# Quillboltcode/VLM-CLIP

Measured on AMD Instinct MI355X. Metric: image-text pairs/sec, ViT-B/16 contrastive step, 1/2/4/8 GPUs; MFMA % peak, higher is better.
Workload: dtype bf16

## Files before the change

vlm-clip_amd/csrc/gemm.hip:

```cpp
#include "common.h"
#include "internal.h"
#include <algorithm>
#include <cstring>
#include <type_traits>
#include <cstdlib>

#include "gemm_common.h"

namespace {
using namespace cmg;

template <bool AK, bool BKM, typename OutT, int EPI>
__global__ __launch_bounds__(NTHR, 2) void gemm_bf16_kernel(GemmP p) {
  extern __shared__ __attribute__((aligned(16))) char smem[];
  const int t = threadIdx.x, lane = t & 63, wave = t >> 6;
  const int wm = wave >> 1, wn = wave & 1;
  const int tile = xcd_remap(blockIdx.x, p.ntiles);
  const int tm = tile / p.tiles_n, tn = tile - tm * p.tiles_n;
  const int m0 = tm * BM, n0 = tn * BN;
  const int kbeg = blockIdx.y * p.k_per_split;
  const int kend = min(p.K, kbeg + p.k_per_split);
  const int nk = (kend - kbeg + BK - 1) / BK;

  Stager<AK> sa;
// ... 938 lines not shown
  }
}

template <bool AK, bool BKM, typename OutT, int EPI>
void launch_bf16(const GemmP& p, int splits, hipStream_t s) {
  hipLaunchKernelGGL((gemm_bf16_kernel<AK, BKM, OutT, EPI>), dim3(p.ntiles, splits), dim3(NTHR), 65536, s, p);
}

template <bool AK, bool BKM, typename OutT, int EPI, bool BG, int VAR>
void launch256v(const GemmP& p, int splits, hipStream_t s, float* bias_grad) {
  (void)lds_optin((const void*)gemm256_kernel<AK, BKM, OutT, EPI, BG, VAR>, 131072);
  hipLaunchKernelGGL((gemm256_kernel<AK, BKM, OutT, EPI, BG, VAR>), dim3(p.ntiles * splits), dim3(NT2), 131072, s,
                     p, bias_grad);
}
template <bool AK, bool BKM, typename OutT, int EPI, bool BG, int PPV>
void launch_ppv(const GemmP& p, int splits, hipStream_t s, float* bias_grad) {
  (void)lds_optin((const void*)gemm_pp_kernel<AK, BKM, OutT, EPI, BG, PPV>, PP_S * PP_STAGE);
  hipLaunchKernelGGL((gemm_pp_kernel<AK, BKM, OutT, EPI, BG, PPV>), dim3(p.ntiles * splits), dim3(NT2),
                     PP_S * PP_STAGE, s, p, bias_grad);
}
int num_cus() {
  static int n[64] = {0};
  int dev = 0;
  (void)hipGetDevice(&dev);
  dev &= 63;
  if (!n[dev]) {
    int c = 0;
    if (hipDeviceGetAttribute(&c, hipDeviceAttributeMultiprocessorCount, dev) != hipSuccess || c <= 0) c = 256;
    n[dev] = c;
  }
  return n[dev];
}
#ifdef CLIPMI_GEMM_EXPERIMENTS
template <bool AK, bool BKM, typename OutT, int EPI>
void launch_pps(const GemmP& p, hipStream_t s) {
  (void)lds_optin((const void*)gemm_pps_kernel<AK, BKM, OutT, EPI>, PP_S * PP_STAGE);
  const int grid = std::min(p.ntiles, num_cus());
  hipLaunchKernelGGL((gemm_pps_kernel<AK, BKM, OutT, EPI>), dim3(grid), dim3(NT2), PP_S * PP_STAGE, s, p);
}
template <bool BKM, typename OutT, int EPI>
void launch_hp(const GemmP& p, hipStream_t s) {
  (void)lds_optin((const void*)gemm_hp_kernel<BKM, OutT, EPI>, 131072);
  hipLaunchKernelGGL((gemm_hp_kernel<BKM, OutT, EPI>), dim3(p.ntiles), dim3(NT2), 131072, s, p);
}
#endif
template <bool AK, bool BKM, typename OutT, int EPI, bool BG>
void launch256(const GemmP& p, int splits, hipStream_t s, float* bias_grad) {
#ifdef CLIPMI_GEMM_EXPERIMENTS
  if (p.var == 10 && !BG && !p.ws && splits == 1) {
    launch_pps<AK, BKM, OutT, EPI>(p, s);
    return;
  }
  if constexpr (AK && !BG) {
    if (p.var == 11 && !p.ws && splits == 1) {
      launch_hp<BKM, OutT, EPI>(p, s);
      return;
    }
  }
  switch (p.var) {
    case 2: launch256v<AK, BKM, OutT, EPI, BG, 0>(p, splits, s, bias_grad); return;
    case 3: launch256v<AK, BKM, OutT, EPI, BG, 2>(p, splits, s, bias_grad); return;
    case 12: launch_ppv<AK, BKM, OutT, EPI, BG, 8>(p, splits, s, bias_grad); return;
    case 13: launch_ppv<AK, BKM, OutT, EPI, BG, 16>(p, splits, s, bias_grad); return;
    case 14: launch_ppv<AK, BKM, OutT, EPI, BG, 20>(p, splits, s, bias_grad); return;
    case 15: launch_ppv<AK, BKM, OutT, EPI, BG, 32>(p, splits, s, bias_grad); return;
    case 16: launch_ppv<AK, BKM, OutT, EPI, BG, 64>(p, splits, s, bias_grad); return;
    case 5: launch_ppv<AK, BKM, OutT, EPI, BG, 1>(p, splits, s, bias_grad); return;
    case 6: launch_ppv<AK, BKM, OutT, EPI, BG, 2>(p, splits, s, bias_grad); return;
    case 7: launch_ppv<AK, BKM, OutT, EPI, BG, 3>(p, splits, s, bias_grad); return;
    case 8: launch_ppv<AK, BKM, OutT, EPI, BG, 4>(p, splits, s, bias_grad); return;
    default: break;
  }
#endif
  if (p.var == 4) launch256v<AK, BKM, OutT, EPI, BG, 3>(p, splits, s, bias_grad);
  else launch_ppv<AK, BKM, OutT, EPI, BG, 0>(p, splits, s, bias_grad);
}

constexpr int E_B = CLIPMI_EPI_BIAS, E_R = CLIPMI_EPI_RESID, E_Q = CLIPMI_EPI_QGELU, E_G = CLIPMI_EPI_GELU;
constexpr int E_P = CLIPMI_EPI_STORE_PRE, E_DQ = CLIPMI_EPI_DQGELU, E_DG = CLIPMI_EPI_DGELU, E_BETA = CLIPMI_EPI_BETA;
constexpr int E_DA = CLIPMI_EPI_STORE_DACT, E_MA = CLIPMI_EPI_MUL_AUX;

bool w4_x3() {
  const char* e = getenv("CLIPMI_GEMM_X3_W4");
  return !(e && e[0] == '0');
}

const char* dispatch256(const GemmP& p, int splits, hipStream_t s, bool f32o, int sel, int flags, float* bg) {
  if (sel == 0 && (p.ws || (f32o && flags == E_BETA))) {
    if (p.var == 28 || p.var == 32) {
      if (const char* l = dispatch_w4_wgrad(p, splits, s, flags, bg)) return l;
    }
    if (p.ws) {
      if (bg) launch256<false, false, float, 0, true>(p, splits, s, bg);
      else launch256<false, false, float, 0, false>(p, splits, s, bg);
      return "gemm256_wgrad_splitk";
    }
    if (bg) launch256<false, false, float, E_BETA, true>(p, splits, s, bg);
    else launch256<false, false, float, E_BETA, false>(p, splits, s, bg);
    return "gemm256_wgrad";
  }
  if (bg) return nullptr;
  const bool w4_pf = p.var == 0 && sel == 2 && (flags == E_MA || (flags == 0 && p.K <= 768));
  const bool w4_default = p.var == 0 && (p.K >= 1536 || flags == E_MA);
  if ((w4_default || w4_pf || p.var == 20 || (p.var >= 22 && p.var <= 25 && p.dbg) || p.var == 28 || p.var == 32) &&
      !f32o && !p.ws && splits == 1 && (sel == 3 || sel == 2)) {
    GemmP q = p;
    const int dm = (p.var == 32 || w4_pf) ? 102 : (p.var == 28 || w4_default) ? 100 : p.var >= 22 ? 21 - p.var : 1;
    if (const char* l = dispatch_w4(q, s, sel == 3, flags, dm)) return l;
  }
  if (f32o && !p.ws && splits == 1 && sel == 3) {
    if ((w4_default || p.var == 28) && (flags == E_B || flags == (E_B | E_R) || flags == 0 || (p.x3o && w4_x3()))) {
      if (const char* l = dispatch_w4_f32(p, s, flags, true)) return l;
    }
    switch (flags) {
      case E_B: launch256<true, true, float, E_B, false>(p, splits, s, bg); return "gemm256_fwd_bias_f32";
      case E_B | E_R: launch256<true, true, float, E_B | E_R, false>(p, splits, s, bg); return "gemm256_fwd_bias_resid_f32";
      case 0: launch256<true, true, float, 0, false>(p, splits, s, bg); return "gemm256_fwd_f32";
      case E_B | E_Q | E_DA: launch256<true, true, float, E_B | E_Q | E_DA, false>(p, splits, s, bg); return "gemm256_fwd_bias_qgelu_dact_f32";
      case E_B | E_Q: launch256<true, true, float, E_B | E_Q, false>(p, splits, s, bg); return "gemm256_fwd_bias_qgelu_f32";
      default: break;
    }
  }
  if (f32o && !p.ws && splits == 1 && sel == 2) {
    if ((w4_default || p.var == 28) && (flags == 0 || (p.x3o && w4_x3()))) {
      if (const char* l = dispatch_w4_f32(p, s, flags, false)) return l;
    }
    switch (flags) {
      case 0: launch256<true, false, float, 0, false>(p, splits, s, bg); return "gemm256_dgrad_f32";
      case E_MA: launch256<true, false, float, E_MA, false>(p, splits, s, bg); return "gemm256_dgrad_mulaux_f32";
      default: break;
    }
  }
  if (sel == 3 && !f32o) {
    switch (flags) {
      case E_B: launch256<true, true, bf16, E_B, false>(p, splits, s, bg); return "gemm256_fwd_bias";
      case E_B | E_R: launch256<true, true, bf16, E_B | E_R, false>(p, splits, s, bg); return "gemm256_fwd_bias_resid";
      case E_B | E_Q | E_P: launch256<true, true, bf16, E_B | E_Q | E_P, false>(p, splits, s, bg); return "gemm256_fwd_bias_qgelu_pre";
      case E_B | E_Q | E_DA: launch256<true, true, bf16, E_B | E_Q | E_DA, false>(p, splits, s, bg); return "gemm256_fwd_bias_qgelu_dact";
      case E_B | E_Q: launch256<true, true, bf16, E_B | E_Q, false>(p, splits, s, bg); return "gemm256_fwd_bias_qgelu";
      case 0: launch256<true, true, bf16, 0, false>(p, splits, s, bg); return "gemm256_fwd";
      default: break;
    }
  }
  if (sel == 2 && !f32o) {
    switch (flags) {
      case 0: launch256<true, false, bf16, 0, false>(p, splits, s, bg); return "gemm256_dgrad";
      case E_DQ: launch256<true, false, bf16, E_DQ, false>(p, splits, s, bg); return "gemm256_dgrad_dqgelu";
      case E_MA: launch256<true, false, bf16, E_MA, false>(p, splits, s, bg); return "gemm256_dgrad_mulaux";
      default: break;
    }
  }
  return nullptr;
}

const char* dispatch_bf16(const GemmP& p, int splits, hipStream_t s, bool f32o, int sel, int flags) {
  if (p.ws) {
    if (sel == 0) { launch_bf16<false, false, float, 0>(p, splits, s); return "gemm_wgrad_splitk"; }
    launch_bf16<true, true, float, -1>(p, splits, s);
    return "gemm_generic";
  }
  if (sel == 3 && !f32o) {
    switch (flags) {
      case E_B: launch_bf16<true, true, bf16, E_B>(p, splits, s); return "gemm_fwd_bias";
      case E_B | E_R: launch_bf16<true, true, bf16, E_B | E_R>(p, splits, s); return "gemm_fwd_bias_resid";
      case E_B | E_Q | E_P: launch_bf16<true, true, bf16, E_B | E_Q | E_P>(p, splits, s); return "gemm_fwd_bias_qgelu_pre";
      case E_B | E_Q: launch_bf16<true, true, bf16, E_B | E_Q>(p, splits, s); return "gemm_fwd_bias_qgelu";
// ... 239 lines not shown
            ((uintptr_t)d->residual % 16 == 0) && ((uintptr_t)d->aux % 16 == 0);
    p.vec8 = d->c_dtype == CLIPMI_BF16 && d->N % 8 == 0 && d->ldc % 8 == 0 && d->ldr % 8 == 0 && d->ldaux % 8 == 0 &&
             ((uintptr_t)d->C % 16 == 0) && ((uintptr_t)d->residual % 16 == 0) && ((uintptr_t)d->aux % 16 == 0) &&
             ((uintptr_t)d->bias % 16 == 0);
    const double flops = 2.0 * d->M * d->N * d->K;
    ProfScope ps(s, nullptr, 0.0);
    const char* label = dispatch_fp8(p, s, d->c_dtype == CLIPMI_F32, q8o, d->flags);
    if (!label) return clipmi_invalid("fp8 output: supported epilogue flags are bias + quick_gelu");
    ps.finish(label, flops);
    CLIPMI_CHECK_LAUNCH();
    return CLIPMI_OK;
  }
  const bool bf = d->ab_dtype == CLIPMI_BF16;
  CLIPMI_REQUIRE(bf || d->ab_dtype == CLIPMI_F32, "ab_dtype");
  if (d->M == 0 || d->N == 0) return CLIPMI_OK;
  CLIPMI_REQUIRE(bf == false || d->b_kmajor || d->N % 8 == 0, "row-major B needs N % 8 == 0");
  CLIPMI_REQUIRE(d->c_dtype == CLIPMI_F32 || d->c_dtype == CLIPMI_BF16, "c_dtype");

  if (bf) {
    CLIPMI_REQUIRE(!d->a_kmajor || d->K % 8 == 0, "k-major A needs K % 8 == 0");
    CLIPMI_REQUIRE(!d->b_kmajor || d->K % 8 == 0, "k-major B needs K % 8 == 0");
    CLIPMI_REQUIRE(d->a_kmajor || d->M % 8 == 0, "row-major A needs M % 8 == 0");
    CLIPMI_REQUIRE(d->a_kmajor || d->M >= 8, "M >= 8");
    CLIPMI_REQUIRE(((uintptr_t)d->A & 15) == 0 && ((uintptr_t)d->B & 15) == 0, "A/B must be 16-byte aligned");
    CLIPMI_REQUIRE((d->lda % 8) == 0 && (d->ldb % 8) == 0, "lda/ldb must be multiples of 8");
  }
  int splits = d->split_k > 1 ? d->split_k : 1;
  GemmP p;
  memset(&p, 0, sizeof(p));
  p.M = d->M; p.N = d->N; p.K = d->K;
  p.A = d->A; p.lda = d->lda; p.B = d->B; p.ldb = d->ldb;
  p.C = d->C; p.ldc = d->ldc; p.bias = d->bias; p.res = d->residual; p.ldr = d->ldr;
  p.aux = d->aux; p.ldaux = d->ldaux; p.alpha = d->alpha; p.flags = d->flags;
  p.bias_f32 = d->bias_dtype == CLIPMI_F32;
  p.ws = nullptr;
  p.bws = nullptr;
  p.x3o = x3o;
  p.colp = colp;
  static const int env_var = [] {
    const char* e = getenv("CLIPMI_GEMM_VAR");
    return e ? atoi(e) : -1;
  }();
  static const int env_wvar = [] {
    const char* e = getenv("CLIPMI_GEMM_WVAR");
    return e ? atoi(e) : -1;
  }();
  const bool wlayout = !d->a_kmajor && !d->b_kmajor;
  const int evar = wlayout ? env_wvar : env_var;
  p.raster = raster_rows();
  p.dbg = gemm_stamp_buffer();
  p.stagger = 0;
  p.first_round = num_cus();
  if (d->force_small_tile >= 100 && d->force_small_tile < 200) {
    p.var = 9;
    p.stagger = d->force_small_tile % 100;
  } else if (d->force_small_tile >= 2) p.var = d->force_small_tile;
  else if (evar >= 0 && d->force_small_tile == 0) p.var = evar;
  else p.var = wlayout ? 28 : 0;
  p.vec = (d->ldc % 4 == 0) && (d->ldr % 4 == 0) && (d->ldaux % 4 == 0) && ((uintptr_t)d->C % 16 == 0) &&
          ((uintptr_t)d->residual % 16 == 0) && ((uintptr_t)d->aux % 16 == 0);
  p.vec8 = d->c_dtype == CLIPMI_BF16 && d->N % 8 == 0 && d->ldc % 8 == 0 && d->ldr % 8 == 0 && d->ldaux % 8 == 0 &&
           ((uintptr_t)d->C % 16 == 0) && ((uintptr_t)d->residual % 16 == 0) && ((uintptr_t)d->aux % 16 == 0) &&
           ((uintptr_t)d->bias % 16 == 0);
  const bool kok = (!d->a_kmajor || d->K % 64 == 0) && (!d->b_kmajor || d->K % 64 == 0);
  const bool use256 = bf && kok && ((d->M >= 256 && d->N >= 128) || d->bias_grad) && d->force_small_tile != 1;
  CLIPMI_REQUIRE(!d->bias_grad || use256, "bias_grad fusion needs the 256 kernel (bf16, wgrad layout)");
  CLIPMI_REQUIRE(!x3o || (use256 && splits == 1), "x3out: needs the 256-tile kernels (M >= 256, N >= 128, K % 64 == 0)");
  const int tile = bf ? (use256 ? BT : BM) : FT;
  const int kstep = bf ? BK : FK;
  if (splits > 1) {
    CLIPMI_REQUIRE(d->c_dtype == CLIPMI_F32, "split_k needs fp32 C");
    CLIPMI_REQUIRE((d->flags & ~CLIPMI_EPI_BETA) == 0, "split_k supports only the beta flag");
    CLIPMI_REQUIRE(d->workspace && d->workspace_bytes >= (int64_t)splits * d->M * (d->N + (d->bias_grad ? 1 : 0)) * 4,
                   "split_k workspace too small (split_k * M * (N + bias_grad ? 1 : 0) floats)");
    int per = (d->K + splits - 1) / splits;
    per = (per + kstep - 1) / kstep * kstep;
    splits = (d->K + per - 1) / per;
    p.k_per_split = per;
    p.ws = (float*)d->workspace;
    if (d->bias_grad) p.bws = p.ws + (int64_t)splits * d->M * d->N;
  } else {
    p.k_per_split = d->K > 0 ? d->K : 1;
  }
  p.tiles_n = (d->N + tile - 1) / tile;
  p.ntiles = p.tiles_n * ((d->M + tile - 1) / tile);
  const double flops = 2.0 * d->M * d->N * d->K;
  if (bf) {
    const bool f32o = d->c_dtype == CLIPMI_F32 || p.ws;
    const int sel = (d->a_kmajor ? 2 : 0) | (d->b_kmajor ? 1 : 0);
    ProfScope ps(s, nullptr, 0.0);
    const char* label = nullptr;
    if (use256) {
      GemmP q = p;
      q.tiles_n = (d->N + BT - 1) / BT;
      q.ntiles = q.tiles_n * ((d->M + BT - 1) / BT);
      if (wlayout && !getenv("CLIPMI_RASTER") && q.tiles_n > q.ntiles / q.tiles_n) q.raster = q.ntiles / q.tiles_n;
      label = dispatch256(q, splits, s, f32o, sel, d->flags, d->bias_grad);
      CLIPMI_REQUIRE(label || !x3o, "x3out: no image-output kernel for these flags");
    }
    if (!label) {
      CLIPMI_REQUIRE(!d->bias_grad, "bias_grad needs the wgrad layout (both operands row-major in k)");
      GemmP q = p;
      q.tiles_n = (d->N + BM - 1) / BM;
      q.ntiles = q.tiles_n * ((d->M + BM - 1) / BM);
      label = dispatch_bf16(q, splits, s, f32o, sel, d->flags);
    }
    CLIPMI_REQUIRE(label, "no kernel for this GEMM");
    ps.finish(label, flops);
  } else {
    ProfScope ps(s, nullptr, 0.0);
    if (d->c_dtype == CLIPMI_F32 || p.ws)
      hipLaunchKernelGGL(gemm_f32_kernel<float>, dim3(p.ntiles, splits), dim3(256), 0, s, p, d->a_kmajor, d->b_kmajor);
    else
      hipLaunchKernelGGL(gemm_f32_kernel<bf16>, dim3(p.ntiles, splits), dim3(256), 0, s, p, d->a_kmajor, d->b_kmajor);
    ps.finish("gemm_f32", flops);
  }
  CLIPMI_CHECK_LAUNCH();
  if (p.ws) {
    const int64_t total = (int64_t)d->M * d->N;
    const int beta = (d->flags & CLIPMI_EPI_BETA) ? 1 : 0;
    if (d->N % 4 == 0 && d->ldc % 4 == 0 && ((uintptr_t)d->C & 15) == 0 && ((uintptr_t)p.ws & 15) == 0) {
      DeferredReduce r;
      memset(&r, 0, sizeof(r));
      r.kind = 1;
      r.ws = p.ws; r.C = (float*)d->C; r.ldc = d->ldc; r.M = d->M; r.N = d->N; r.splits = splits;
      r.alpha = d->alpha; r.beta = beta; r.bws = p.bws; r.bias_grad = d->bias_grad;
      DeferredReduce* slot = deferred_slot();
      if (slot && slot->kind == 0) *slot = r;
      else CLIPMI_TRY(launch_deferred(s, r));
    } else {
      const unsigned nblk = (unsigned)std::min<int64_t>((total + 255) / 256, 8192);
      hipLaunchKernelGGL(splitk_reduce_kernel, dim3(nblk), dim3(256), 0, s,
                         p.ws, (float*)d->C, d->ldc, d->M, d->N, splits, d->alpha, beta);
      if (p.bws)
        hipLaunchKernelGGL(bias_partials_reduce_kernel, dim3((d->M + 255) / 256), dim3(256), 0, s, p.bws,
                           d->bias_grad, d->M, splits);
    }
    CLIPMI_CHECK_LAUNCH();
  }
  return CLIPMI_OK;
}
}

extern "C" int clipmi_gemm(void* stream, const clipmi_gemm_desc* d) { return gemm_impl(stream, d, 0, nullptr); }

namespace {
__global__ __launch_bounds__(256) void fold_rows4_kernel(const float* part, int P, int N, int per, float* out) {
  const int c = (blockIdx.x * 256 + threadIdx.x) * 4;
  if (c >= N) return;
  const int r0 = blockIdx.y * per, r1 = min(P, r0 + per);
  f32x4 acc = f32x4{0.f, 0.f, 0.f, 0.f};
  int r = r0;
  for (; r + 8 <= r1; r += 8) {
    f32x4 v[8];
#pragma unroll
    for (int j = 0; j < 8; ++j) v[j] = *(const f32x4*)(part + (int64_t)(r + j) * N + c);
#pragma unroll
    for (int j = 0; j < 8; ++j) acc += v[j];
  }
  for (; r < r1; ++r) acc += *(const f32x4*)(part + (int64_t)r * N + c);
  *(f32x4*)(out + (int64_t)blockIdx.y * N + c) = acc;
}
constexpr int X3_FOLD = 64;
int x3out_parts(int M) { return (M + 127) / 128; }
}

// ... 91 lines not shown
```

vlm-clip_amd/csrc/gemm_common.h:

```cpp
#pragma once
#include "common.h"
#include "internal.h"
#include <algorithm>
#include <type_traits>

namespace cmg {

constexpr int BM = 128, BN = 128, BK = 64, NTHR = 256;
constexpr int E8_B = CLIPMI_EPI_BIAS, E8_R = CLIPMI_EPI_RESID, E8_Q = CLIPMI_EPI_QGELU;

struct GemmP {
  int M, N, K;
  const void* A; int64_t lda;
  const void* B; int64_t ldb;
  void* C; int64_t ldc;
  const void* bias; const void* res; int64_t ldr;
  void* aux; int64_t ldaux;
  float alpha; int flags; int bias_f32;
  int k_per_split; float* ws;
  int tiles_n, ntiles;
  int vec;
  int var;
  int vec8;
  int stagger, first_round;
  const uint8_t* a_scale; const uint8_t* b_scale;
  uint8_t* c_scale;
  int raster;
  float* bws;
  unsigned long long* dbg;
  int* dyn;
  int nb2;
  int64_t bsa1, bsa2, bsb1, bsb2, bsc1, bsc2;
  DeferredReduce red;
  int x3o;
  float* colp;
};

unsigned long long* gemm_stamp_buffer();

__device__ __forceinline__ void tile_coords(const GemmP& p, int tile, int& tm, int& tn) {
  if (p.raster > 0) {
    const int g = p.raster, tiles_m = p.ntiles / p.tiles_n;
    const int grp = tile / (g * p.tiles_n);
    const int rem = tile - grp * g * p.tiles_n;
    const int rows = min(g, tiles_m - grp * g);
    tn = rem / rows;
    tm = grp * g + (rem - tn * rows);
  } else {
    tm = tile / p.tiles_n;
    tn = tile - tm * p.tiles_n;
  }
}

__device__ __forceinline__ float ld_bias(const GemmP& p, int n) {
  return p.bias_f32 ? ((const float*)p.bias)[n] : (float)((const bf16*)p.bias)[n];
}

template <typename OutT>
__device__ __forceinline__ void ld4(const OutT* p, float v[4], int nv, bool vec) {
  if (vec) { load4(p, v); return; }
#pragma unroll
  for (int j = 0; j < 4; ++j) v[j] = j < nv ? to_f32(p[j]) : 0.f;
}
template <typename OutT>
__device__ __forceinline__ void st4(OutT* p, const float v[4], int nv, bool vec) {
  if (vec) { store4(p, v); return; }
#pragma unroll
  for (int j = 0; j < 4; ++j)
    if (j < nv) p[j] = from_f32<OutT>(v[j]);
}

template <typename OutT, int EPI>
__device__ __forceinline__ void epilogue4(const GemmP& p, int m, int n, float v[4]) {
  const int f = EPI >= 0 ? EPI : p.flags;
  const int nv = min(4, p.N - n);
  const bool vec = p.vec && nv == 4;
#pragma unroll
  for (int j = 0; j < 4; ++j) v[j] *= p.alpha;
  if (f & CLIPMI_EPI_BIAS) {
#pragma unroll
    for (int j = 0; j < 4; ++j) v[j] += j < nv ? ld_bias(p, n + j) : 0.f;
  }
  if (f & CLIPMI_EPI_STORE_PRE) st4((OutT*)p.aux + (int64_t)m * p.ldaux + n, v, nv, vec);
  if (f & CLIPMI_EPI_STORE_DACT) {
    float d[4];
#pragma unroll
    for (int j = 0; j < 4; ++j) d[j] = (f & CLIPMI_EPI_QGELU) ? quick_gelu_grad(v[j]) : gelu_erf_grad(v[j]);
    st4((OutT*)p.aux + (int64_t)m * p.ldaux + n, d, nv, vec);
  }
  if (f & CLIPMI_EPI_QGELU) {
#pragma unroll
    for (int j = 0; j < 4; ++j) v[j] = quick_gelu(v[j]);
  } else if (f & CLIPMI_EPI_GELU) {
#pragma unroll
    for (int j = 0; j < 4; ++j) v[j] = gelu_erf(v[j]);
  }
  if (f & (CLIPMI_EPI_DQGELU | CLIPMI_EPI_DGELU)) {
    float a[4];
    ld4((const OutT*)p.aux + (int64_t)m * p.ldaux + n, a, nv, vec);
    if (f & CLIPMI_EPI_DQGELU) {
#pragma unroll
      for (int j = 0; j < 4; ++j) v[j] *= quick_gelu_grad(a[j]);
    } else {
#pragma unroll
      for (int j = 0; j < 4; ++j) v[j] *= gelu_erf_grad(a[j]);
    }
// ... 484 lines not shown
#pragma unroll
  for (int part = 0; part < NPART; ++part) {
    const int c = part >> 1, h = part & 1;
    u32x4 aux2[4][2];
#pragma unroll
    for (int ii = 0; ii < 4; ++ii) {
      const int i = h * 4 + ii;
#pragma unroll
      for (int jp = 0; jp < 2; ++jp) {
        float v[8];
        if constexpr (AR) __builtin_amdgcn_sched_barrier(0);
#pragma unroll
        for (int r = 0; r < 4; ++r) {
          const auto sw = __builtin_amdgcn_permlane16_swap(__float_as_uint(acc[c][i][2 * jp][r]),
                                                           __float_as_uint(acc[c][i][2 * jp + 1][r]), false, false);
          v[r] = __uint_as_float(sw[0]) * p.alpha + bv[c][jp][r];
          v[r + 4] = __uint_as_float(sw[1]) * p.alpha + bv[c][jp][r + 4];
        }
        float xin[8], w2[8];
        if (HIN) unpack8(xr[part % PD][ii][jp], xin);
#pragma unroll
        for (int r = 0; r < 8; ++r) {
          if (HPRE) w2[r] = v[r];
          if (HQ) {
            const float sg = qg_sigmoid(v[r]);
            if (HDA) {
              const float tq = 1.702f * v[r];
              w2[r] = fmaf(sg, fmaf(-tq, sg, tq), sg);
            }
            v[r] *= sg;
          }
          if (HG) {
            if (HDA) w2[r] = gelu_erf_grad(v[r]);
            v[r] = gelu_erf(v[r]);
          }
          if (HDQ) v[r] *= quick_gelu_grad(xin[r]);
          if (HDG) v[r] *= gelu_erf_grad(xin[r]);
          if (HMA) v[r] *= xin[r];
          if (HR || HBETA) v[r] += xin[r];
        }
        if (H2)
          aux2[ii][jp] = __builtin_bit_cast(u32x4, bf16x8{(bf16)w2[0], (bf16)w2[1], (bf16)w2[2], (bf16)w2[3],
                                                           (bf16)w2[4], (bf16)w2[5], (bf16)w2[6], (bf16)w2[7]});
        *LDS_PTR(bf16x8, st + stage_off(ii * 16 + mlane, (32 * jp + coff) >> 3)) =
            bf16x8{(bf16)v[0], (bf16)v[1], (bf16)v[2], (bf16)v[3], (bf16)v[4], (bf16)v[5], (bf16)v[6], (bf16)v[7]};
      }
    }
    if (HIN && part + PD < NPART) load_in(part + PD, xr[part % PD]);
    asm volatile("s_waitcnt lgkmcnt(0)" ::: "memory");
    u32x4 o[8];
#pragma unroll
    for (int it = 0; it < 8; ++it) o[it] = *LDS_PTR(const u32x4, st + stage_off(it * 8 + (lane >> 3), lane & 7));
    asm volatile("s_waitcnt lgkmcnt(0)" ::: "memory");
    if (H2) {
#pragma unroll
      for (int ii = 0; ii < 4; ++ii)
#pragma unroll
        for (int jp = 0; jp < 2; ++jp) *LDS_PTR(u32x4, st + stage_off(ii * 16 + mlane, (32 * jp + coff) >> 3)) = aux2[ii][jp];
    }
    const int r0 = mb + h * 64 + (lane >> 3), col = nb + 64 * c + (lane & 7) * 8;
    auto store_rows = [&](bf16* base, int64_t ld, const u32x4 (&rows)[8]) {
      bf16* out = base + (int64_t)r0 * ld + col;
      const int64_t step = 8 * ld;
      if (full) {
#pragma unroll
        for (int it = 0; it < 8; ++it) st16_out((u32x4*)(out + it * step), rows[it]);
      } else {
#pragma unroll
        for (int it = 0; it < 8; ++it)
          if (r0 + it * 8 < p.M && col < p.N) st16_out((u32x4*)(out + it * step), rows[it]);
      }
    };
    store_rows((bf16*)p.C, p.ldc, o);
    if (H2) {
      asm volatile("s_waitcnt lgkmcnt(0)" ::: "memory");
#pragma unroll
      for (int it = 0; it < 8; ++it) o[it] = *LDS_PTR(const u32x4, st + stage_off(it * 8 + (lane >> 3), lane & 7));
      asm volatile("s_waitcnt lgkmcnt(0)" ::: "memory");
      store_rows((bf16*)p.aux, p.ldaux, o);
    }
  }
}

template <int EPI, bool AR = false>
__device__ __forceinline__ void epilogue_x3img(const GemmP& p, f32x4 (&acc)[8][4], int mb, int nb, int lane) {
#pragma clang fp contract(off)
  constexpr bool HB = EPI & CLIPMI_EPI_BIAS, HQ = EPI & CLIPMI_EPI_QGELU;
  constexpr bool HDA = EPI & CLIPMI_EPI_STORE_DACT, HMA = EPI & CLIPMI_EPI_MUL_AUX;
  const int q = lane >> 4, mlane = lane & 15;
  const int coff = 16 * (q & 1) + 8 * (q >> 1);
  const int64_t seg = p.N;
  const bool p1 = p.x3o == 2;
  float bv[2][8];
#pragma unroll
  for (int jp = 0; jp < 2; ++jp) {
    const int n = min(nb + 32 * jp + coff, p.N - 8);
#pragma unroll
    for (int r = 0; r < 8; ++r) bv[jp][r] = 0.f;
    if (HB) {
      if (p.bias_f32) {
        load4((const float*)p.bias + n, bv[jp]);
        load4((const float*)p.bias + n + 4, bv[jp] + 4);
      } else {
        load8((const bf16*)p.bias + n, bv[jp]);
      }
    }
  }
  float cs[2][8];
#pragma unroll
  for (int jp = 0; jp < 2; ++jp)
#pragma unroll
    for (int r = 0; r < 8; ++r) cs[jp][r] = 0.f;
#pragma unroll
  for (int h = 0; h < 2; ++h) {
    float xin[4][2][8];
    if (HMA) {
#pragma unroll
      for (int ii = 0; ii < 4; ++ii) {
        const int m = min(mb + (h * 4 + ii) * 16 + mlane, p.M - 1);
#pragma unroll
        for (int jp = 0; jp < 2; ++jp) {
          const float* a = (const float*)p.aux + (int64_t)m * p.ldaux + min(nb + 32 * jp + coff, p.N - 8);
          load4(a, xin[ii][jp]);
          load4(a + 4, xin[ii][jp] + 4);
        }
      }
    }
#pragma unroll
    for (int ii = 0; ii < 4; ++ii) {
      const int i = h * 4 + ii;
      const int m = mb + i * 16 + mlane;
#pragma unroll
      for (int jp = 0; jp < 2; ++jp) {
        const int n = nb + 32 * jp + coff;
        float v[8], w2[8];
        if constexpr (AR) __builtin_amdgcn_sched_barrier(0);
#pragma unroll
        for (int r = 0; r < 4; ++r) {
          const auto sw = __builtin_amdgcn_permlane16_swap(__float_as_uint(acc[i][2 * jp][r]),
                                                           __float_as_uint(acc[i][2 * jp + 1][r]), false, false);
          v[r] = __uint_as_float(sw[0]) * p.alpha + bv[jp][r];
          v[r + 4] = __uint_as_float(sw[1]) * p.alpha + bv[jp][r + 4];
        }
#pragma unroll
        for (int r = 0; r < 8; ++r) {
          if (HQ) {
            const float sg = qg_sigmoid(v[r]);
            if (HDA) {
              const float tq = 1.702f * v[r];
              w2[r] = fmaf(sg, fmaf(-tq, sg, tq), sg);
            }
            v[r] *= sg;
          }
          if (HMA) v[r] *= xin[ii][jp][r];
        }
        if (m < p.M && n < p.N) {
          if (HDA) {
            float* a = (float*)p.aux + (int64_t)m * p.ldaux + n;
            store4(a, w2);
            store4(a + 4, w2 + 4);
          }
          bf16x8 hi, lo;
#pragma unroll
          for (int r = 0; r < 8; ++r) {
            hi[r] = (bf16)v[r];
            lo[r] = (bf16)(v[r] - (float)hi[r]);
            cs[jp][r] += v[r];
          }
          bf16* o = (bf16*)p.C + (int64_t)m * p.ldc + n;
          *(bf16x8*)o = hi;
          *(bf16x8*)(o + seg) = p1 ? lo : hi;
          *(bf16x8*)(o + 2 * seg) = p1 ? hi : lo;
        }
      }
    }
  }
  if (p.colp && mb < p.M) {
#pragma unroll
    for (int jp = 0; jp < 2; ++jp) {
#pragma unroll
      for (int r = 0; r < 8; ++r) {
#pragma unroll
        for (int o = 1; o < 16; o <<= 1) cs[jp][r] += __shfl_xor(cs[jp][r], o, 64);
      }
      const int n = nb + 32 * jp + coff;
      if (mlane == 0 && n < p.N) {
        float* c = p.colp + (int64_t)(mb >> 7) * p.N + n;
        store4(c, cs[jp]);
        store4(c + 4, cs[jp] + 4);
      }
    }
  }
}

template <typename OutT, int EPI, bool AR = false>
__device__ __forceinline__ void finish256(const GemmP& p, f32x4 (&acc)[8][4], int mb, int nb, int lane, int kz,
                                          char* stage = nullptr) {
  constexpr bool FAST = EPI >= 0 && !((EPI & CLIPMI_EPI_RESID) && (EPI & (CLIPMI_EPI_DQGELU | CLIPMI_EPI_DGELU))) &&
                        !((EPI & CLIPMI_EPI_BETA) && (EPI & (CLIPMI_EPI_RESID | CLIPMI_EPI_DQGELU | CLIPMI_EPI_DGELU)));
  constexpr int X3E = EPI & ~CLIPMI_EPI_STORE_DACT;
  if constexpr (std::is_same<OutT, float>::value &&
                (X3E == (CLIPMI_EPI_BIAS | CLIPMI_EPI_QGELU) || EPI == CLIPMI_EPI_MUL_AUX)) {
    if (p.x3o) {
      epilogue_x3img<EPI, AR>(p, acc, mb, nb, lane);
      return;
    }
  }
  constexpr bool NEWF = EPI >= 0 && (EPI & (CLIPMI_EPI_STORE_DACT | CLIPMI_EPI_MUL_AUX));
  if constexpr (NEWF) {
#if !CLIPMI_OLD_EPI
    if constexpr (std::is_same<OutT, bf16>::value) {
      if (stage && !p.ws && p.vec8) {
        epilogue_lds_pipe<EPI, AR, 1>(p, reinterpret_cast<f32x4(&)[1][8][4]>(acc), mb, nb, lane, stage);
        return;
      }
    }
#endif
  } else if constexpr (FAST && std::is_same<OutT, bf16>::value) {
    if (stage && !p.ws && p.vec8) {
#if CLIPMI_OLD_EPI
      epilogue256_lds<EPI < 0 ? 0 : EPI, AR>(p, acc, mb, nb, lane, stage);
#else
      epilogue_lds_pipe<EPI < 0 ? 0 : EPI, AR, 1>(p, reinterpret_cast<f32x4(&)[1][8][4]>(acc), mb, nb, lane, stage);
#endif
      return;
    }
    if (!p.ws && p.vec8) {
      epilogue256_w<EPI < 0 ? 0 : EPI, AR>(p, acc, mb, nb, lane);
      return;
    }
  }
  if (FAST && !NEWF && !p.ws && p.vec && (p.N & 3) == 0) {
    epilogue256<OutT, EPI < 0 ? 0 : EPI, AR>(p, acc, mb, nb, lane);
    return;
  }
#pragma unroll
  for (int i = 0; i < 8; ++i) {
    const int m = mb + i * 16 + (lane & 15);
    if (m >= p.M) continue;
#pragma unroll
    for (int j = 0; j < 4; ++j) {
      const int n = nb + j * 16 + (lane >> 4) * 4;
      if (n >= p.N) continue;
      acc_pin<AR>(acc[i][j]);
      float v[4] = {acc[i][j][0], acc[i][j][1], acc[i][j][2], acc[i][j][3]};
      if (p.ws) st4(p.ws + (int64_t)kz * p.M * p.N + (int64_t)m * p.N + n, v, min(4, p.N - n), p.vec && n + 4 <= p.N);
      else epilogue4<OutT, EPI>(p, m, n, v);
    }
  }
}

template <typename OutT, int EPI, bool AR>
__device__ __forceinline__ void finish256x2(const GemmP& p, f32x4 (&acc)[2][8][4], int mb, int nb, int lane, int kz,
                                            char* stage) {
  constexpr bool FAST = EPI >= 0 && !((EPI & CLIPMI_EPI_RESID) && (EPI & (CLIPMI_EPI_DQGELU | CLIPMI_EPI_DGELU))) &&
                        !((EPI & CLIPMI_EPI_BETA) && (EPI & (CLIPMI_EPI_RESID | CLIPMI_EPI_DQGELU | CLIPMI_EPI_DGELU)));
#if !CLIPMI_OLD_EPI
  if constexpr (FAST && std::is_same<OutT, bf16>::value) {
    if (stage && !p.ws && p.vec8) {
      epilogue_lds_pipe<EPI < 0 ? 0 : EPI, AR, 2>(p, acc, mb, nb, lane, stage);
      return;
    }
  }
#endif
  finish256<OutT, EPI, AR>(p, acc[0], mb, nb, lane, kz, stage);
  finish256<OutT, EPI, AR>(p, acc[1], mb, nb + 64, lane, kz, stage);
}

typedef __attribute__((ext_vector_type(8))) int i32x8;
typedef __attribute__((ext_vector_type(16))) float f32x16;
typedef __attribute__((ext_vector_type(2))) float f32x2;

template <int EPI, int NI = 8>
__device__ __forceinline__ void epilogue_q8(const GemmP& p, f32x4 (&acc)[NI][4], int mb, int nb, int lane) {
  constexpr bool HB = EPI & CLIPMI_EPI_BIAS, HQ = EPI & CLIPMI_EPI_QGELU, HG = EPI & CLIPMI_EPI_GELU;
  const int q = lane >> 4, mlane = lane & 15;
  const int coff = 16 * (q & 1) + 8 * (q >> 1);
  uint8_t* out = (uint8_t*)p.C;
  const int nsb = p.N >> 5;
  float bv[2][8];
#pragma unroll
  for (int jp = 0; jp < 2; ++jp) {
    const int n = min(nb + 32 * jp + coff, p.N - 8);
#pragma unroll
    for (int r = 0; r < 8; ++r) bv[jp][r] = 0.f;
    if (HB) {
      if (p.bias_f32) {
        load4((const float*)p.bias + n, bv[jp]);
        load4((const float*)p.bias + n + 4, bv[jp] + 4);
      } else {
        load8((const bf16*)p.bias + n, bv[jp]);
      }
    }
  }
#pragma unroll
  for (int i = 0; i < NI; ++i) {
    const int m = mb + i * 16 + mlane;
    uint32_t w[2][2];
    int ex[2];
#pragma unroll
    for (int jp = 0; jp < 2; ++jp) {
      f32x2 v2[4];
#pragma unroll
      for (int r = 0; r < 4; ++r) {
        const auto sw = __builtin_amdgcn_permlane16_swap(__float_as_uint(acc[i][2 * jp][r]),
                                                         __float_as_uint(acc[i][2 * jp + 1][r]), false, false);
        v2[r] = __builtin_elementwise_fma(f32x2{__uint_as_float(sw[0]), __uint_as_float(sw[1])},
                                          f32x2{p.alpha, p.alpha}, f32x2{bv[jp][r], bv[jp][r + 4]});
      }
      float am = 0.f;
#pragma unroll
      for (int r = 0; r < 4; ++r) {
        if (HQ) {
          const f32x2 z = v2[r] * f32x2{-1.702f * 1.4426950408889634f, -1.702f * 1.4426950408889634f};
          const f32x2 d = f32x2{__builtin_amdgcn_exp2f(z[0]), __builtin_amdgcn_exp2f(z[1])} + f32x2{1.0f, 1.0f};
          v2[r] = v2[r] * f32x2{__builtin_amdgcn_rcpf(d[0]), __builtin_amdgcn_rcpf(d[1])};
        }
        if (HG) v2[r] = f32x2{gelu_erf(v2[r][0]), gelu_erf(v2[r][1])};
        am = fmaxf(am, fmaxf(fabsf(v2[r][0]), fabsf(v2[r][1])));
      }
      am = fmaxf(am, __shfl_xor(am, 16, 64));
      am = fmaxf(am, __shfl_xor(am, 32, 64));
      ex[jp] = mx_exponent(am);
      const float inv = ldexpf(1.0f, -ex[jp]);
#pragma unroll
      for (int r = 0; r < 4; ++r) v2[r] = v2[r] * f32x2{inv, inv};
      int pk = __builtin_amdgcn_cvt_pk_fp8_f32(v2[0][0], v2[1][0], 0, false);
      w[jp][0] = (uint32_t)__builtin_amdgcn_cvt_pk_fp8_f32(v2[2][0], v2[3][0], pk, true);
      pk = __builtin_amdgcn_cvt_pk_fp8_f32(v2[0][1], v2[1][1], 0, false);
      w[jp][1] = (uint32_t)__builtin_amdgcn_cvt_pk_fp8_f32(v2[2][1], v2[3][1], pk, true);
    }
    const auto s0 = __builtin_amdgcn_permlane32_swap(w[0][0], w[1][0], false, false);
    const auto s1 = __builtin_amdgcn_permlane32_swap(w[0][1], w[1][1], false, false);
    const int col = nb + 16 * q;
    if (m < p.M && col < p.N) *(u32x4*)(out + (int64_t)m * p.ldc + col) = u32x4{s0[0], s1[0], s0[1], s1[1]};
    if (q == 0 && m < p.M) {
      const int sb = (nb >> 5);
      if ((nsb & 1) == 0 && nb + 64 <= p.N) {
        *(uint16_t*)(p.c_scale + (int64_t)m * nsb + sb) = (uint16_t)((ex[0] + 127) | ((ex[1] + 127) << 8));
      } else {
        p.c_scale[(int64_t)m * nsb + sb] = (uint8_t)(ex[0] + 127);
        if (nb + 32 < p.N) p.c_scale[(int64_t)m * nsb + sb + 1] = (uint8_t)(ex[1] + 127);
      }
    }
  }
}

// ... 7 lines not shown
```

Measured before the change: 7817.

## Add LDS-staged pipelined fp32 epilogue with buffer stores and prefetched residual

Adds an fp32-output epilogue for the 256-tile GEMM. Accumulators are transposed through LDS with permlane16 swaps so each lane writes full 128-bit rows, and stores go through buffer resource descriptors. Residual loads are prefetched a configurable number of parts ahead. It is meant to replace the scattered 4-float per-lane stores of fp32 bias/residual GEMM outputs with coalesced wide stores and to hide residual-read latency. It is enabled by default behind an env var and only runs when alignment and full-tile conditions hold, at the cost of extra LDS traffic and register pressure from the prefetch buffers.

```diff
diff --git a/vlm-clip_amd/csrc/gemm.hip b/vlm-clip_amd/csrc/gemm.hip
--- a/vlm-clip_amd/csrc/gemm.hip
+++ b/vlm-clip_amd/csrc/gemm.hip
@@ -1044,6 +1044,11 @@
 
 bool w4_x3() {
   const char* e = getenv("CLIPMI_GEMM_X3_W4");
+  return !(e && e[0] == '0');
+}
+
+bool epi_f32_pipe() {
+  const char* e = getenv("CLIPMI_EPI_F32_PIPE");
   return !(e && e[0] == '0');
 }
 
@@ -1449,6 +1454,9 @@
   } else {
     p.k_per_split = d->K > 0 ? d->K : 1;
   }
+  p.f32pipe = d->c_dtype == CLIPMI_F32 && !p.ws && !x3o && !colp && epi_f32_pipe() && d->N % 8 == 0 && d->ldc % 4 == 0 &&
+              d->ldr % 4 == 0 && d->ldc < (1 << 22) && d->ldr < (1 << 22) && ((uintptr_t)d->C % 16 == 0) && ((uintptr_t)d->residual % 16 == 0) &&
+              ((uintptr_t)d->bias % 16 == 0);
   p.tiles_n = (d->N + tile - 1) / tile;
   p.ntiles = p.tiles_n * ((d->M + tile - 1) / tile);
   const double flops = 2.0 * d->M * d->N * d->K;
diff --git a/vlm-clip_amd/csrc/gemm_common.h b/vlm-clip_amd/csrc/gemm_common.h
--- a/vlm-clip_amd/csrc/gemm_common.h
+++ b/vlm-clip_amd/csrc/gemm_common.h
@@ -22,6 +22,7 @@
   int vec;
   int var;
   int vec8;
+  int f32pipe;
   int stagger, first_round;
   const uint8_t* a_scale; const uint8_t* b_scale;
   uint8_t* c_scale;
@@ -672,6 +673,99 @@
   }
 }
 
+#ifndef CLIPMI_EPI_F32_PD
+#define CLIPMI_EPI_F32_PD 2
+#endif
+__device__ __forceinline__ __amdgpu_buffer_rsrc_t wave_rsrc(const void* base, uint32_t bytes) {
+  const uint64_t b = (uint64_t)base;
+  const uint32_t hi = __builtin_amdgcn_readfirstlane((uint32_t)(b >> 32)), lo = __builtin_amdgcn_readfirstlane((uint32_t)b);
+  const uint64_t u = ((uint64_t)hi << 32) | (uint64_t)lo;
+  return __builtin_amdgcn_make_buffer_rsrc((void*)u, (short)0, __builtin_amdgcn_readfirstlane(bytes), 0x00020000);
+}
+__device__ __forceinline__ int stage_off_f32(int r, int k) { return r * 256 + ((k ^ ((r & 11) | ((r >> 1) & 4))) << 4); }
+
+template <int EPI, bool AR, int NC>
+__device__ __forceinline__ void epilogue_lds_pipe_f32(const GemmP& p, f32x4 (&acc)[NC][8][4], int mb, int nb, int lane,
+                                                      char* st) {
+  constexpr bool HB = EPI & CLIPMI_EPI_BIAS, HR = EPI & CLIPMI_EPI_RESID;
+  static_assert((EPI & ~(CLIPMI_EPI_BIAS | CLIPMI_EPI_RESID)) == 0, "bias and residual only");
+  constexpr int NPART = 4 * NC;
+  const int q = lane >> 4, mlane = lane & 15;
+  const int coff = 16 * (q & 1) + 8 * (q >> 1);
+  const int rr = lane >> 4, rk = lane & 15;
+  float bv[NC][2][8];
+#pragma unroll
+  for (int c = 0; c < NC; ++c)
+#pragma unroll
+    for (int jp = 0; jp < 2; ++jp) {
+      const int n = nb + 64 * c + 32 * jp + coff;
+#pragma unroll
+      for (int r = 0; r < 8; ++r) bv[c][jp][r] = 0.f;
+      if (HB) {
+        if (p.bias_f32) {
+          load4((const float*)p.bias + n, bv[c][jp]);
+          load4((const float*)p.bias + n + 4, bv[c][jp] + 4);
+        } else {
+          load8((const bf16*)p.bias + n, bv[c][jp]);
+        }
+      }
+    }
+  const __amdgpu_buffer_rsrc_t rres =
+      wave_rsrc((const float*)p.res + (int64_t)mb * p.ldr + nb, HR ? (uint32_t)((127 * p.ldr + 64 * NC) * 4) : 0u);
+  const __amdgpu_buffer_rsrc_t rout = wave_rsrc((float*)p.C + (int64_t)mb * p.ldc + nb, (uint32_t)((127 * p.ldc + 64 * NC) * 4));
+  const int roff = (rr * (int)p.ldr + 4 * rk) * 4, woff = (rr * (int)p.ldc + 4 * rk) * 4;
+  constexpr int PD = CLIPMI_EPI_F32_PD < NPART ? CLIPMI_EPI_F32_PD : NPART;
+  f32x4 xr[PD][8];
+  auto load_in = [&](int part, f32x4 (&x)[8]) {
+    const int c = part >> 2, h = part & 3;
+#pragma unroll
+    for (int it = 0; it < 8; ++it)
+      x[it] = __builtin_bit_cast(
+          f32x4, __builtin_amdgcn_raw_buffer_load_b128(rres, roff, ((32 * h + 4 * it) * (int)p.ldr + 64 * c) * 4, 0));
+  };
+  if (HR) {
+#pragma unroll
+    for (int d = 0; d < PD; ++d) load_in(d, xr[d]);
+  }
+#pragma unroll
+  for (int part = 0; part < NPART; ++part) {
+    const int c = part >> 2, h = part & 3;
+#pragma unroll
+    for (int ii = 0; ii < 2; ++ii) {
+      const int i = h * 2 + ii;
+#pragma unroll
+      for (int jp = 0; jp < 2; ++jp) {
+        float v[8];
+        if constexpr (AR) __builtin_amdgcn_sched_barrier(0);
+#pragma unroll
+        for (int r = 0; r < 4; ++r) {
+          const auto sw = __builtin_amdgcn_permlane16_swap(__float_as_uint(acc[c][i][2 * jp][r]),
+                                                           __float_as_uint(acc[c][i][2 * jp + 1][r]), false, false);
+          v[r] = __uint_as_float(sw[0]) * p.alpha + bv[c][jp][r];
+          v[r + 4] = __uint_as_float(sw[1]) * p.alpha + bv[c][jp][r + 4];
+        }
+        const int k = (32 * jp + coff) >> 2;
+        *LDS_PTR(f32x4, st + stage_off_f32(ii * 16 + mlane, k)) = f32x4{v[0], v[1], v[2], v[3]};
+        *LDS_PTR(f32x4, st + stage_off_f32(ii * 16 + mlane, k + 1)) = f32x4{v[4], v[5], v[6], v[7]};
+      }
+    }
+    asm volatile("s_waitcnt lgkmcnt(0)" ::: "memory");
+    f32x4 o[8];
+#pragma unroll
+    for (int it = 0; it < 8; ++it) o[it] = *LDS_PTR(const f32x4, st + stage_off_f32(4 * it + rr, rk));
+    asm volatile("s_waitcnt lgkmcnt(0)" ::: "memory");
+    if (HR) {
+#pragma unroll
+      for (int it = 0; it < 8; ++it) o[it] += xr[part % PD][it];
+      if (part + PD < NPART) load_in(part + PD, xr[part % PD]);
+    }
+#pragma unroll
+    for (int it = 0; it < 8; ++it)
+      __builtin_amdgcn_raw_buffer_store_b128(__builtin_bit_cast(u32x4, o[it]), rout, woff,
+                                             ((32 * h + 4 * it) * (int)p.ldc + 64 * c) * 4, 0);
+  }
+}
+
 template <int EPI, bool AR = false>
 __device__ __forceinline__ void epilogue_x3img(const GemmP& p, f32x4 (&acc)[8][4], int mb, int nb, int lane) {
 #pragma clang fp contract(off)
@@ -782,6 +876,10 @@
     }
   }
 }
+
+template <typename OutT, int EPI>
+constexpr bool F32P = std::is_same<OutT, float>::value &&
+                      (EPI == 0 || EPI == CLIPMI_EPI_BIAS || EPI == (CLIPMI_EPI_BIAS | CLIPMI_EPI_RESID));
 
 template <typename OutT, int EPI, bool AR = false>
 __device__ __forceinline__ void finish256(const GemmP& p, f32x4 (&acc)[8][4], int mb, int nb, int lane, int kz,
@@ -820,6 +918,12 @@
       return;
     }
   }
+  if constexpr (F32P<OutT, EPI>) {
+    if (stage && p.f32pipe && mb + 128 <= p.M && nb + 64 <= p.N) {
+      epilogue_lds_pipe_f32<EPI, AR, 1>(p, reinterpret_cast<f32x4(&)[1][8][4]>(acc), mb, nb, lane, stage);
+      return;
+    }
+  }
   if (FAST && !NEWF && !p.ws && p.vec && (p.N & 3) == 0) {
     epilogue256<OutT, EPI < 0 ? 0 : EPI, AR>(p, acc, mb, nb, lane);
     return;
@@ -853,6 +957,12 @@
     }
   }
 #endif
+  if constexpr (F32P<OutT, EPI>) {
+    if (stage && p.f32pipe && mb + 128 <= p.M && nb + 128 <= p.N) {
+      epilogue_lds_pipe_f32<EPI, AR, 2>(p, acc, mb, nb, lane, stage);
+      return;
+    }
+  }
   finish256<OutT, EPI, AR>(p, acc[0], mb, nb, lane, kz, stage);
   finish256<OutT, EPI, AR>(p, acc[1], mb, nb + 64, lane, kz, stage);
 }
```

Result: no change. 7857 (median of 6 runs) (+0.5%).
